# apple/ml-stable-diffusion

Hardware: AMD Instinct MI355X
Metric: diffusion iter/s (UNet steps/s), SD2.1-base 512x512 fp16 (higher is better)
Workload: dtype fp16; 1 GPU; BASELINE config 2: SD2.1-base (865.9 M-parameter UNet), random-init, denoising iteration at 512x512 (64x64 latents), CFG batch 2 per prompt, DDIM, device-resident loop; unet=sd21-base, latent=64, attention=ORIGINAL, prompts_per_gpu=1, global_batch=2, hip_graph=True, parallelism=dp1 (independent prompts per rank, no data-path collective)

## Files before the change

include/sd_mi355x.h:

```cpp
#ifndef SD_MI355X_H
#define SD_MI355X_H

#include <stddef.h>
#include <stdint.h>

#ifdef __cplusplus
extern "C" {
#endif

typedef enum sd_status {
  SD_OK = 0,
  SD_ERR_INVALID_ARGUMENT = -1,
  SD_ERR_NOT_FOUND = -2,
  SD_ERR_HIP = -3,
  SD_ERR_UNSUPPORTED = -4,
  SD_ERR_INTERNAL = -5
} sd_status;

typedef enum sd_dtype { SD_F16 = 0, SD_F32 = 1 } sd_dtype;

typedef enum sd_attention_impl {
  SD_ATTN_ORIGINAL = 0,
  SD_ATTN_SPLIT_EINSUM = 1,
  SD_ATTN_SPLIT_EINSUM_V2 = 2
// ... 140 lines not shown
                           const float* gn_bias, void* conv_out, void* out, int B, int Cin, int H, int W, int Cout, int ksize,
                           int groups, float eps, int silu, int tile, int producer_stats, int* entries, int iters, float* ms);
int sd_op_conv2d_groupnorm_proj(const void* x, const void* w, const float* bias, const void* res, const float* gn_weight,
                                const float* gn_bias, const void* proj_w, const float* proj_bias, void* conv_out, void* out, int B,
                                int Cin, int H, int W, int Cout, int ksize, int Nproj, int groups, float eps, int fold, int tile,
                                int* entries, int iters, float* ms);
int sd_op_conv2d_groupnorm_conv3x3(const void* x, const void* w, const float* bias, const void* res, const float* gn_weight,
                                   const float* gn_bias, const void* w2, const float* bias2, const void* res2, void* conv_out, void* out,
                                   int B, int Cin, int H, int W, int Cout, int ksize, int N2, int groups, float eps, int silu, int fold,
                                   int tile, int staging2, int* entries, int iters, float* ms);
int sd_op_ffn_out_proj(const void* g, const void* w1, const float* b1, const void* res1, const void* w2, const float* b2, const void* res2,
                       void* out, float* gn_sums, int B, int C, int S, int groups, int fused, int iters, float* ms);
int sd_op_fold_linear(const void* wp, const float* bp, const void* w2, const float* b2, void* wm_out, float* bm_out, int N, int J, int K);
int sd_op_cross_attention_fused(const void* x, const float* ln_weight, const float* ln_bias, const void* wq, const void* k,
                                const void* v, void* out, int B, int heads, int Sq, int Sk, float eps, int nst, int iters,
                                float* ms);
int sd_op_cross_attention_block(const void* x, const float* ln_weight, const float* ln_bias, const void* wq, const void* k, const void* v,
                                const void* wo, const float* bo, const void* a1, const void* wo1, const float* bo1, void* out, int B, int heads,
                                int Sq, int Sk, float eps, int fused, int iters, float* ms);
int sd_op_geglu(const void* x, const void* w, const float* bias, void* out, int M, int C, int N2, int iters, float* ms);
int sd_op_geglu_ln(const void* x, const float* ln_weight, const float* ln_bias, const void* w, const float* bias, void* out, int M, int C,
                   int N2, float eps, int kernel, int iters, float* ms);
int sd_op_qkv_ln(const void* x, const float* ln_weight, const float* ln_bias, const void* w, void* out_qk, void* out_vt, int B, int HW, int C,
                 float eps, float q_scale, int vt_perm, int kernel, int iters, float* ms);
int sd_op_gn_proj_qkv(const void* x_in, const void* conv_w, const float* gn_weight, const float* gn_bias, const void* proj_w,
                      const float* proj_bias, const float* ln_weight, const float* ln_bias, const void* wqkv, void* out_h, void* out_qk,
                      void* out_vt, int B, int H, int W, int C, int groups, float gn_eps, float ln_eps, float q_scale, int vt_perm, int fused,
                      int* entries, int iters, float* ms);
int sd_op_timestep_embedding(const float* t, float* out, int n, int dim, int flip_sin_to_cos, float freq_shift);
int sd_op_posterior_noise(const float* moments, const float* eps, const float* noise, float* out, int Cz, int h, int w, int n_images,
                          float scale_factor, float sa, float sb, int iters, float* ms);
int sd_op_conv_plan(int ksize, int stride, int up, int C0, int C1, int N, int B, int Ho, int Wo, int out_mode, int flags, int n_trans,
                    int n_twins, int gnf_groups, int tile, int staging, int splitk, int copies, int* plan, unsigned long long* workspace_bytes);
int sd_numpy_randn(uint32_t seed, double* out, size_t n);
int sd_torch_randn(uint32_t seed, double* out, size_t n);
int sd_philox_randn(uint64_t seed, uint32_t offset, double* out, size_t n);
int sd_calibrate(int device, float* out9);
int sd_selftest_mfma(void);

typedef struct sd_safety_checker_config {
  int32_t batch, image_size , patch_size , hidden_size, intermediate_size,
          num_hidden_layers, num_attention_heads, projection_dim, num_concepts ,
          num_special , hidden_act ;
  float layer_norm_eps;
  int32_t use_graph;
} sd_safety_checker_config;
typedef struct sd_safety_checker sd_safety_checker;
int sd_safety_checker_create(const sd_safety_checker_config* cfg, const sd_weights* w, int device, sd_safety_checker** out);
void sd_safety_checker_destroy(sd_safety_checker* c);
size_t sd_safety_checker_device_bytes(const sd_safety_checker* c);
int sd_safety_checker_run(sd_safety_checker* c, const void* clip_input, float adjustment, float* has_nsfw,
                          float* concept_scores, float* image_embeds, float* last_hidden_state, int flags);
float sd_safety_checker_last_ms(const sd_safety_checker* c);
int sd_op_vit_attention(const void* qkv, void* out, int B, int S, int heads, int d, int iters, float* ms);
int sd_op_safety_head(const float* image_embeds, const float* concept_embeds, const float* special_embeds,
                      const float* concept_w, const float* special_w, float adjustment, int B, int P,
                      int n_concepts, int n_special, float* has_nsfw, float* concept_scores);

#ifdef __cplusplus
}
#endif
#endif
```

ml-stable-diffusion_amd/csrc/capi_ops.cpp:

```cpp
#include <algorithm>
#include <climits>
#include <cmath>
#include <cstring>
#include <initializer_list>

#include "capi_util.h"
#include "conv_plan.h"
#include "weight_prep.h"

namespace sd {
namespace {

const half_t* f16(const void* p) { return reinterpret_cast<const half_t*>(p); }

half_t* upload_nhwc(Scratch& sc, const void* x, int B, int C, int H, int W) {
  const half_t* src = f16(x);
  std::vector<half_t> t((size_t)B * C * H * W);
  for (int b = 0; b < B; ++b)
    for (int c = 0; c < C; ++c)
      for (int p = 0; p < H * W; ++p) t[((size_t)b * H * W + p) * C + c] = src[((size_t)b * C + c) * H * W + p];
  return sc.dev<half_t>(t.size(), t.data());
}
half_t* upload_tokens(Scratch& sc, const void* x, int B, int C, int S) { return upload_nhwc(sc, x, B, C, 1, S); }

// ... 564 lines not shown
    cd.gnf_groups = groups;
    SD_REQUIRE(conv_fast_path_ok(cd), kInvalidArgument, "conv2d_groupnorm_conv3x3: the second conv must run on the MFMA path");
    const bool can_fold = fold && silu && conv_gn_loader_ok(cd);
    SD_REQUIRE(!fold || can_fold, kUnsupported, "conv2d_groupnorm_conv3x3: the halo loader cannot normalise C=%d groups=%d @%dx%d", Cout, groups, H, W);
    cd.gnf_groups = 0;
    ConvWorkspace ws = workspace_for(sc, {d, cd});
    int n_entries = 0;
    sc.timed(iters, ms, [&] {
      n_entries = launch_conv(d, ws, sc.stream);
      ConvDesc cc = cd;
      if (fold && n_entries >= 1 && n_entries <= 128) {
        fold_groupnorm(cc, dconv, partial, dgw, dgb, eps, groups, n_entries);
        cc.gnf_silu = silu ? 1 : 0;
      } else {
        launch_groupnorm(dconv, Cout, nullptr, 0, partial, dgw, dgb, dnorm, B, H * W, groups, eps, silu ? 1 : 0, sc.stream, n_entries);
        cc.x0 = dnorm;
      }
      launch_conv(cc, ws, sc.stream);
    });
    if (entries) *entries = (fold && n_entries >= 1 && n_entries <= 128) ? n_entries : 0;
    if (conv_out) download_nchw(dconv, conv_out, B, Cout, H, W);
    download_nchw(dy, out, B, N2, H, W);
  });
}

int sd_op_cross_attention_fused(const void* x, const float* ln_weight, const float* ln_bias, const void* wq, const void* k,
                                const void* v, void* out, int B, int heads, int Sq, int Sk, float eps, int nst, int iters,
                                float* ms) {
  return guarded([&] {
    SD_REQUIRE(x && ln_weight && ln_bias && wq && k && v && out, kInvalidArgument, "NULL argument");
    const int C = heads * 64;
    SD_REQUIRE(B > 0 && heads > 0 && xattn_fused_ok(C, heads, Sq, Sk), kUnsupported,
               "cross_attention_fused: heads %d x 64 channels, Sq %d, Sk %d (<= 96)", heads, Sq, Sk);
    Scratch sc;
    const int ldv = (Sk + 7) / 8 * 8;
    const FoldedProj fq = upload_ln_folded(sc, wq, nullptr, ln_weight, ln_bias, C, C, false);
    XAttnDesc d;
    d.x = upload_tokens(sc, x, B, C, Sq);
    d.wq = fq.w;
    d.bias = fq.bias;
    d.colsum = fq.colsum;
    d.k = upload_tokens(sc, k, B, C, Sk);
    d.vt = upload_vt(sc, v, B, C, Sk, ldv, false);
    half_t* o = sc.dev<half_t>((size_t)B * Sq * C);
    d.out = o;
    d.M = B * Sq; d.C = C; d.S = Sq; d.L = Sk; d.ldv = ldv; d.heads = heads;
    d.ln_eps = eps;
    d.nst = nst;
    sc.timed(iters, ms, [&] { launch_xattn_fused(d, sc.stream); });
    download_tokens(o, out, B, C, Sq);
  });
}

int sd_op_cross_attention_block(const void* x, const float* ln_weight, const float* ln_bias, const void* wq, const void* k, const void* v,
                                const void* wo, const float* bo, const void* a1, const void* wo1, const float* bo1, void* out, int B, int heads,
                                int Sq, int Sk, float eps, int fused, int iters, float* ms) {
  return guarded([&] {
    SD_REQUIRE(x && ln_weight && ln_bias && wq && k && v && wo && bo && out, kInvalidArgument, "NULL argument");
    const bool pre = a1 != nullptr;
    SD_REQUIRE(!pre || (wo1 && bo1), kInvalidArgument, "cross_attention_block: a1 needs wo1 and bo1");
    const int C = heads * 64;
    SD_REQUIRE(B > 0 && heads > 0 && xattn_fused_ok(C, heads, Sq, Sk), kUnsupported,
               "cross_attention_block: heads %d x 64 channels, Sq %d, Sk %d (<= 96)", heads, Sq, Sk);
    SD_REQUIRE(!fused || (xattn_out_ok(C, heads, Sq, Sk) && (!pre || heads == 5)), kUnsupported,
               "cross_attention_block: the one-launch form takes 5 or 10 heads (with a1: 5) and Sq %% 32 == 0 (heads %d, Sq %d)", heads, Sq);
    Scratch sc;
// ... 371 lines not shown
    ConvDesc d;
    d.x0 = d.w = ph;
    d.C0 = C0;
    if (C1 > 0) d.x1 = ph, d.C1 = C1;
    d.B = B; d.Ho = Ho; d.Wo = Wo; d.Hi = Ho * stride / up; d.Wi = Wo * stride / up;
    d.ksize = ksize; d.stride = stride; d.up = up; d.N = N; d.out_mode = out_mode;
    if (flags & 1) d.ln_colsum = present;
    if (flags & 2) d.temb = present;
    if (flags & 4) d.res = ph;
    if (flags & 8) d.gn_partial = const_cast<float*>(present), d.gn_groups = 32;
    if (flags & 16) d.bias = present;
    if (flags & 32) d.pad = 0;
    if (n_trans > 0) d.out_t = const_cast<half_t*>(ph), d.n_trans = n_trans, d.ldT = Ho * Wo;
    d.n_twins = n_twins;
    if (gnf_groups > 0) {
      d.gnf_partial = d.gnf_gamma = d.gnf_beta = present;
      d.gnf_groups = gnf_groups;
      d.gnf_entries = 1;
      d.gnf_silu = ksize == 3 ? 1 : 0;
    }
    d.tile = tile; d.staging = staging; d.splitk = splitk;
    const ConvWeightCopies c = conv_plan_copies(d);
    if (copies < 0) copies = (c.wstream ? 1 : 0) | (c.wsgemm ? 2 : 0) | (c.bvgemm ? 4 : 0);
    if (copies & 1) d.w_tiled = ph;
    if (copies & 2) d.w_ws = ph;
    if (copies & 4) d.w_bv = ph;
    const ConvPlan p = conv_plan(d);
    plan[0] = p.tile; plan[1] = p.staging; plan[2] = p.splitk; plan[3] = p.slab ? 1 : 0;
    plan[4] = c.wstream ? 1 : 0; plan[5] = c.wsgemm ? 1 : 0; plan[6] = c.bvgemm ? 1 : 0;
    *workspace_bytes = p.workspace_bytes;
  });
}

int sd_op_timestep_embedding(const float* t, float* out, int n, int dim, int flip_sin_to_cos, float freq_shift) {
  return guarded([&] {
    SD_REQUIRE(t && out && n > 0 && dim > 0 && dim % 2 == 0, kInvalidArgument, "bad arguments");
    SD_REQUIRE(flip_sin_to_cos == 1, kUnsupported, "flip_sin_to_cos=False is not on the path");
    Scratch sc;
    float* dt = sc.dev<float>(n, t);
    float* dout = sc.dev<float>((size_t)n * dim);
    std::vector<float> f = timestep_freq_table(dim, freq_shift);
    float* df = sc.dev<float>(f.size(), f.data());
    launch_timestep_embedding(dt, df, dout, n, dim, sc.stream);
    SD_HIP(hipStreamSynchronize(sc.stream));
    SD_HIP(hipMemcpy(out, dout, (size_t)n * dim * sizeof(float), hipMemcpyDeviceToHost));
  });
}

int sd_op_posterior_noise(const float* moments, const float* eps, const float* noise, float* out, int Cz, int h, int w, int n_images,
                          float scale_factor, float sa, float sb, int iters, float* ms) {
  return guarded([&] {
    SD_REQUIRE(moments && eps && noise && out, kInvalidArgument, "NULL argument");
    SD_REQUIRE(Cz > 0 && h > 0 && w > 0 && n_images > 0, kInvalidArgument, "posterior_noise: Cz=%d h=%d w=%d n_images=%d", Cz, h, w, n_images);
    Scratch sc;
    const size_t n = (size_t)Cz * h * w, total = (size_t)n_images * n, guard = 256;
    float* dm = sc.dev<float>(2 * n, moments);
    float* de = sc.dev<float>(n, eps);
    float* dn = sc.dev<float>(total, noise);
    float* dout = sc.dev<float>(total + guard);
    SD_HIP(hipMemset(dout, 0xff, (total + guard) * sizeof(float)));
    sc.timed(iters, ms, [&] { launch_posterior_noise(dm, de, dn, dout, n, n_images, scale_factor, sa, sb, sc.stream); });
    SD_HIP(hipStreamSynchronize(sc.stream));
    std::vector<uint32_t> g(guard);
    SD_HIP(hipMemcpy(g.data(), dout + total, guard * sizeof(float), hipMemcpyDeviceToHost));
    for (uint32_t v : g) SD_REQUIRE(v == 0xffffffffu, kInternal, "posterior_noise wrote behind its %zu outputs", total);
    SD_HIP(hipMemcpy(out, dout, total * sizeof(float), hipMemcpyDeviceToHost));
// ... 48 lines not shown
```

ml-stable-diffusion_amd/csrc/kernels.h:

```cpp
#pragma once
#include "sd_common.h"

namespace sd {

enum OutMode : int {
  kOutHalf = 0,
  kOutHalfT = 1,
  kOutGeglu = 2,
};

struct GnTwin {
  half_t* y = nullptr;
  int ld = 0, c_off = 0;
  int cpg = 0;
  const float* gamma = nullptr;
  const float* beta = nullptr;
  float eps = 1e-5f;
  int silu = 0;
};

struct ConvDesc {
  const half_t* x0 = nullptr;
  const half_t* x1 = nullptr;
  int C0 = 0, C1 = 0;
// ... 112 lines not shown
  int variant = 0;
  int vt_perm = 0;
  int q_prescaled = 0;
  float* sk_part = nullptr;
  size_t sk_part_bytes = 0;
  unsigned* sk_cnt = nullptr;
  int sk_cnt_n = 0;
  int sk_force = 0;
  int sk_upw = 0;
};
inline float attention_q_prescale(int d) { return 1.4426950408889634f / sqrtf((float)d); }
void launch_attention(const AttnDesc& d, hipStream_t s);
bool attention_supported(int d);
bool attention8_ok(const AttnDesc& d);
bool attention8_shape_ok(int d, int Sq, int Sk);
void launch_attention8(const AttnDesc& d, hipStream_t s);
bool attention8_sk_scratch(const AttnDesc& d, size_t* part_bytes, int* n_counters);

struct XAttnDesc {
  const half_t* x = nullptr;
  const half_t* wq = nullptr;
  const float* bias = nullptr;
  const float* colsum = nullptr;
  const half_t* k = nullptr;
  const half_t* vt = nullptr;
  half_t* out = nullptr;
  int M = 0, C = 0, S = 0, L = 0, ldv = 0, heads = 0;
  float ln_eps = 1e-5f;
  int impl = kAttnOriginal;
  int nst = 0;
};
bool xattn_fused_ok(int C, int heads, int S, int L);
void launch_xattn_fused(const XAttnDesc& d, hipStream_t s);

struct XAttnOutDesc {
  const half_t* x = nullptr;
  const half_t* wq_t = nullptr;
  const float* q_bias = nullptr;
  const float* q_colsum = nullptr;
  const half_t* k = nullptr;
  const half_t* vt = nullptr;
  const half_t* wo_t = nullptr;
  const float* o_bias = nullptr;
  half_t* out = nullptr;
  int M = 0, C = 0, S = 0, L = 0, ldv = 0, heads = 0;
  float ln_eps = 1e-5f;
  int impl = kAttnOriginal;
  const half_t* h0 = nullptr;
  const half_t* wo1_t = nullptr;
  const float* o1_bias = nullptr;
};
struct GnProjQkvDesc {
  const half_t* x = nullptr;
  const float* gn_partial = nullptr;
  const float* gn_gamma = nullptr;
  const float* gn_beta = nullptr;
  int gn_entries = 0, gn_groups = 32;
  float gn_eps = 1e-6f;
  const half_t* wp_t = nullptr;
  const float* p_bias = nullptr;
  half_t* h = nullptr;
  const half_t* wqkv_t = nullptr;
  const float* qkv_bias = nullptr;
  const float* qkv_colsum = nullptr;
  float ln_eps = 1e-5f;
  half_t* qk = nullptr;
// ... 112 lines not shown
```

ml-stable-diffusion_amd/csrc/xattn.hip:

```cpp
#include "kernels.h"

namespace sd {
namespace {

constexpr int BK = 64;
constexpr int XBM = 128;
constexpr int XD = 64;
constexpr int XKEYS = 96;
constexpr int KROW = XD + 4;
constexpr int VROW = XKEYS + 4;

struct XAttnArgs {
  const half_t* x;
  const half_t* wq;
  const float* bias;
  const float* colsum;
  const half_t* k;
  const half_t* vt;
  half_t* out;
  int M, C, S, L, ldv, heads;
  float ln_eps, scale_log2;
};

__device__ __forceinline__ float xor32_sumf(float v) {
  const unsigned u = __float_as_uint(v);
  const auto r = __builtin_amdgcn_permlane32_swap(u, u, false, false);
  const unsigned r0 = r[0], r1 = r[1];
  return __uint_as_float(r0) + __uint_as_float(r1);
}
__device__ __forceinline__ float xor32_maxf(float v) {
  const unsigned u = __float_as_uint(v);
  const auto r = __builtin_amdgcn_permlane32_swap(u, u, false, false);
  const unsigned r0 = r[0], r1 = r[1];
  return fmaxf(__uint_as_float(r0), __uint_as_float(r1));
}

constexpr size_t xattn_lds_bytes(int nst) {
  return (size_t)nst * (XBM + XD) * BK * 2 + (size_t)XKEYS * KROW * 2 + (size_t)XD * VROW * 2 + 2 * XD * sizeof(float);
}

template <int NST>
__global__ __launch_bounds__(256, xattn_lds_bytes(NST) <= 80 * 1024 ? 2 : 1) void xattn_fused_kernel(XAttnArgs a) {
  constexpr int XR = XBM / 32, WR = XD / 32;
  extern __shared__ __attribute__((aligned(16))) char smem[];
  half_t* Xs = reinterpret_cast<half_t*>(smem);
  half_t* Ws = Xs + NST * XBM * BK;
  half_t* Ks = Ws + NST * XD * BK;
  half_t* Vs = Ks + XKEYS * KROW;
  float* sconst = reinterpret_cast<float*>(Vs + XD * VROW);

  const int tid = threadIdx.x, lane = tid & 63;
  const int wave = __builtin_amdgcn_readfirstlane(tid >> 6);
  const int l31 = lane & 31, hi = lane >> 5;

  const int tps = (a.S + XBM - 1) / XBM;
  const int nwg = (a.M / a.S) * tps * a.heads;
  int bid = blockIdx.x;
  {
    const int q = nwg >> 3, r = nwg & 7, xcd = bid & 7, idx = bid >> 3;
    bid = ((xcd < r) ? xcd * (q + 1) : r * (q + 1) + (xcd - r) * q) + idx;
  }
  const int mt = bid / a.heads, h = bid - mt * a.heads;
  const int b = mt / tps;
  const int m_blk = b * a.S + (mt - b * tps) * XBM;
  const int rows_valid = min(XBM, a.S - (mt - b * tps) * XBM);
  const int nk = a.C / BK;

  const half8 zero8 = {0, 0, 0, 0, 0, 0, 0, 0};
  half8 kreg[3], vreg[3];
  {
    const half_t* kb = a.k + (size_t)b * a.L * a.C + (size_t)h * XD;
    const half_t* vb = a.vt + ((size_t)b * a.C + (size_t)h * XD) * a.ldv;
#pragma unroll
    for (int i = 0; i < 3; ++i) {
      const int idx = tid + i * 256;
      const int row = idx >> 3, ch = idx & 7;
      kreg[i] = (row < a.L) ? *reinterpret_cast<const half8*>(kb + (size_t)row * a.C + ch * 8) : zero8;
    }
#pragma unroll
    for (int i = 0; i < 3; ++i) {
      const int idx = tid + i * 256;
      const int row = idx / 12, ch = idx - row * 12;
      vreg[i] = (ch * 8 < a.ldv) ? *reinterpret_cast<const half8*>(vb + (size_t)row * a.ldv + ch * 8) : zero8;
    }
  }
  if (tid < XD) {
    sconst[tid] = a.bias[h * XD + tid];
    sconst[XD + tid] = a.colsum[h * XD + tid];
  }

  const int pchunk = tid & 7, lrow = tid >> 3;
  const int chunk = pchunk ^ ((lrow >> 1) & 7);
  const half_t* xp[XR];
  const half_t* wp[WR];
#pragma unroll
  for (int i = 0; i < XR; ++i) xp[i] = a.x + (size_t)min(m_blk + lrow + 32 * i, a.M - 1) * a.C + chunk * 8;
#pragma unroll
  for (int i = 0; i < WR; ++i) wp[i] = a.wq + (size_t)(h * XD + lrow + 32 * i) * a.C + chunk * 8;
  auto load_tile = [&](int stage) {
    char* xs = reinterpret_cast<char*>(Xs + stage * XBM * BK) + wave * 1024;
    char* ws = reinterpret_cast<char*>(Ws + stage * XD * BK) + wave * 1024;
#pragma unroll
    for (int i = 0; i < XR; ++i) {
      __builtin_amdgcn_global_load_lds((const __attribute__((address_space(1))) void*)xp[i],
                                       (__attribute__((address_space(3))) void*)(xs + i * 4096), 16, 0, 0);
      xp[i] += BK;
    }
#pragma unroll
    for (int i = 0; i < WR; ++i) {
      __builtin_amdgcn_global_load_lds((const __attribute__((address_space(1))) void*)wp[i],
                                       (__attribute__((address_space(3))) void*)(ws + i * 4096), 16, 0, 0);
      wp[i] += BK;
    }
  };

  floatx16 acc[2];
#pragma unroll
  for (int j = 0; j < 2; ++j)
#pragma unroll
    for (int r = 0; r < 16; ++r) acc[j][r] = 0.f;
  float ln_s1 = 0.f, ln_s2 = 0.f;
  const int fsw = (l31 >> 1) & 7;

  constexpr int PER_TILE = XR + WR;
  constexpr int DEPTH = NST - 2;
#pragma unroll
  for (int p = 0; p < NST - 1; ++p)
    if (p < nk) load_tile(p);
  for (int kt = 0; kt < nk; ++kt) {
    const int ahead = nk - 1 - kt;
    const int fly = ahead < DEPTH ? ahead : DEPTH;
    if (DEPTH >= 3 && fly == 3) asm volatile("s_waitcnt vmcnt(%0)\n\ts_barrier" ::"n"((DEPTH >= 3 ? 3 : 0) * PER_TILE) : "memory");
    else if (DEPTH >= 2 && fly == 2) asm volatile("s_waitcnt vmcnt(%0)\n\ts_barrier" ::"n"((DEPTH >= 2 ? 2 : 0) * PER_TILE) : "memory");
    else if (DEPTH >= 1 && fly == 1) asm volatile("s_waitcnt vmcnt(%0)\n\ts_barrier" ::"n"((DEPTH >= 1 ? 1 : 0) * PER_TILE) : "memory");
    else asm volatile("s_waitcnt vmcnt(0)\n\ts_barrier" ::: "memory");
    const int st = kt % NST;
    const half_t* xs = Xs + st * XBM * BK + (wave * 32 + l31) * BK;
    const half_t* ws = Ws + st * XD * BK + l31 * BK;
    half8 xf[4], wf[4][2];
#pragma unroll
    for (int kk = 0; kk < 4; ++kk) {
      const int koff = ((kk * 2 + hi) ^ fsw) * 8;
      xf[kk] = *reinterpret_cast<const half8*>(xs + koff);
#pragma unroll
      for (int j = 0; j < 2; ++j) wf[kk][j] = *reinterpret_cast<const half8*>(ws + j * 32 * BK + koff);
    }
    __builtin_amdgcn_sched_barrier(0);
    if (kt + NST - 1 < nk) load_tile((kt + NST - 1) % NST);
#pragma unroll
    for (int kk = 0; kk < 4; ++kk) {
#pragma unroll
      for (int j = 0; j < 2; ++j) acc[j] = __builtin_amdgcn_mfma_f32_32x32x16_f16(wf[kk][j], xf[kk], acc[j], 0, 0, 0);
      const half2v one2 = {(half_t)1.f, (half_t)1.f};
#pragma unroll
      for (int e = 0; e < 4; ++e) {
        const half2v p2 = {xf[kk][2 * e], xf[kk][2 * e + 1]};
        ln_s2 = __builtin_amdgcn_fdot2(p2, p2, ln_s2, false);
        ln_s1 = __builtin_amdgcn_fdot2(p2, one2, ln_s1, false);
      }
    }
  }

#pragma unroll
  for (int i = 0; i < 3; ++i) {
    const int idx = tid + i * 256;
    const int row = idx >> 3, ch = idx & 7;
    half_t* dst = Ks + row * KROW + ch * 8;
    *reinterpret_cast<half4*>(dst) = half4{kreg[i][0], kreg[i][1], kreg[i][2], kreg[i][3]};
    *reinterpret_cast<half4*>(dst + 4) = half4{kreg[i][4], kreg[i][5], kreg[i][6], kreg[i][7]};
  }
#pragma unroll
  for (int i = 0; i < 3; ++i) {
    const int idx = tid + i * 256;
    const int row = idx / 12, ch = idx - row * 12;
    half_t* dst = Vs + row * VROW + ch * 8;
    *reinterpret_cast<half4*>(dst) = half4{vreg[i][0], vreg[i][1], vreg[i][2], vreg[i][3]};
    *reinterpret_cast<half4*>(dst + 4) = half4{vreg[i][4], vreg[i][5], vreg[i][6], vreg[i][7]};
  }
  __syncthreads();

  half8 qf[2][2];
  {
    const float inv_k = 1.0f / (float)a.C;
    const float s1 = xor32_sumf(ln_s1), s2 = xor32_sumf(ln_s2);
    const float mean = s1 * inv_k;
    const float var = fmaxf(s2 * inv_k - mean * mean, 0.f);
    const float ln_a = rsqrtf(var + a.ln_eps);
    const float ln_b = -ln_a * mean;
#pragma unroll
    for (int j = 0; j < 2; ++j)
#pragma unroll
      for (int q4 = 0; q4 < 4; ++q4) {
        const int nl = j * 32 + 8 * q4 + 4 * hi;
        const floatx4 bb = *reinterpret_cast<const floatx4*>(sconst + nl);
        const floatx4 cs = *reinterpret_cast<const floatx4*>(sconst + XD + nl);
#pragma unroll
        for (int e = 0; e < 4; ++e) {
          const int r = 4 * q4 + e;
          qf[j][r >> 3][r & 7] = (half_t)fmaf(acc[j][r], ln_a, fmaf(ln_b, cs[e], bb[e]));
        }
      }
  }

  floatx16 sacc[3];
#pragma unroll
  for (int kt = 0; kt < 3; ++kt) {
#pragma unroll
    for (int r = 0; r < 16; ++r) sacc[kt][r] = 0.f;
    const half_t* kr = Ks + (kt * 32 + l31) * KROW + 4 * hi;
#pragma unroll
    for (int j = 0; j < 2; ++j)
#pragma unroll
// ... 18 lines not shown
  float ps4[4] = {0.f, 0.f, 0.f, 0.f};
#pragma unroll
  for (int kt = 0; kt < 3; ++kt)
#pragma unroll
    for (int r = 0; r < 16; ++r) {
      const float p = __builtin_amdgcn_exp2f(fmaf(sacc[kt][r], a.scale_log2, -mnew));
      sacc[kt][r] = p;
      ps4[r & 3] += p;
    }
  const float inv = 1.0f / xor32_sumf((ps4[0] + ps4[1]) + (ps4[2] + ps4[3]));

  floatx16 oacc[2];
#pragma unroll
  for (int ct = 0; ct < 2; ++ct)
#pragma unroll
    for (int r = 0; r < 16; ++r) oacc[ct][r] = 0.f;
#pragma unroll
  for (int kt = 0; kt < 3; ++kt)
#pragma unroll
    for (int s2 = 0; s2 < 2; ++s2) {
      half8 pf;
#pragma unroll
      for (int e = 0; e < 8; ++e) pf[e] = (half_t)sacc[kt][s2 * 8 + e];
#pragma unroll
      for (int ct = 0; ct < 2; ++ct) {
        const half_t* vp = Vs + (ct * 32 + l31) * VROW + kt * 32 + s2 * 16 + 4 * hi;
        const half4 v0 = *reinterpret_cast<const half4*>(vp);
        const half4 v1 = *reinterpret_cast<const half4*>(vp + 8);
        const half8 vf = {v0[0], v0[1], v0[2], v0[3], v1[0], v1[1], v1[2], v1[3]};
        oacc[ct] = __builtin_amdgcn_mfma_f32_32x32x16_f16(vf, pf, oacc[ct], 0, 0, 0);
      }
    }

  if (wave * 32 + l31 >= rows_valid) return;
  half_t* orow = a.out + (size_t)(m_blk + wave * 32 + l31) * a.C + (size_t)h * XD;
#pragma unroll
  for (int ct = 0; ct < 2; ++ct)
#pragma unroll
    for (int g = 0; g < 4; ++g) {
      const half4 o = {(half_t)(oacc[ct][4 * g] * inv), (half_t)(oacc[ct][4 * g + 1] * inv),
                       (half_t)(oacc[ct][4 * g + 2] * inv), (half_t)(oacc[ct][4 * g + 3] * inv)};
      *reinterpret_cast<half4*>(orow + ct * 32 + 8 * g + 4 * hi) = o;
    }
}

template <int NST>
void launch_nst(const XAttnArgs& a, hipStream_t s) {
  constexpr size_t lds = xattn_lds_bytes(NST);
  static_assert(lds <= 160 * 1024, "LDS");
  auto k = xattn_fused_kernel<NST>;
  static DynLdsOnce once;
  once.set(k, lds);
  hipLaunchKernelGGL(k, dim3((a.M / a.S) * ((a.S + XBM - 1) / XBM) * a.heads), dim3(256), lds, s, a);
}

}

bool xattn_fused_ok(int C, int heads, int S, int L) {
  static const bool off = tune_env_set("SD_NO_XATTN_FUSED");
  return !off && heads >= 1 && C == heads * XD && C % BK == 0 && S >= 1 && L >= 1 && L <= XKEYS;
}

void launch_xattn_fused(const XAttnDesc& d, hipStream_t s) {
  SD_REQUIRE(xattn_fused_ok(d.C, d.heads, d.S, d.L), kInvalidArgument, "xattn_fused: C=%d heads=%d S=%d L=%d", d.C, d.heads, d.S,
             d.L);
  SD_REQUIRE(d.M % d.S == 0 && d.ldv % 8 == 0 && d.ldv >= d.L && d.ldv <= XKEYS, kInvalidArgument, "xattn_fused: M=%d ldv=%d", d.M,
             d.ldv);
  if (d.impl == kAttnSplitEinsumV2 && d.S >= 512)
    SD_REQUIRE(d.S % 512 == 0, kInvalidArgument, "SPLIT_EINSUM_V2 needs S_q %% 512 == 0 (got %d)", d.S);
  XAttnArgs a{d.x, d.wq, d.bias, d.colsum, d.k, d.vt, d.out, d.M, d.C, d.S, d.L, d.ldv, d.heads, d.ln_eps,
              1.4426950408889634f / sqrtf((float)XD)};
  static const int forced = tune_env_int("SD_XATTN_NST", 0);
  const int nst = forced ? forced : (d.nst ? d.nst : (d.C <= 640 ? 2 : 3));
  if (nst >= 5) launch_nst<5>(a, s);
  else if (nst == 4) launch_nst<4>(a, s);
  else if (nst == 3) launch_nst<3>(a, s);
  else launch_nst<2>(a, s);
  SD_HIP(hipGetLastError());
}

}
```

ml-stable-diffusion_amd/python_hip_stable_diffusion/_lib.py:

```python
import ctypes as C
import os

import numpy as np

_HERE = os.path.dirname(os.path.abspath(__file__))
LIB_PATH = os.environ.get("SD_MI355X_LIB", os.path.join(os.path.dirname(_HERE), "lib", "libsdmi355.so"))

SD_MAX_LEVELS = 6
SD_FLAG_DEVICE_PTRS = 1
ATTENTION_IMPLEMENTATIONS = {"ORIGINAL": 0, "SPLIT_EINSUM": 1, "SPLIT_EINSUM_V2": 2}


class LibraryNotBuilt(ImportError):
    pass


class UNetConfig(C.Structure):
    _fields_ = [
        ("batch", C.c_int32), ("in_channels", C.c_int32), ("out_channels", C.c_int32),
        ("height", C.c_int32), ("width", C.c_int32), ("n_levels", C.c_int32),
        ("block_out_channels", C.c_int32 * SD_MAX_LEVELS),
        ("down_cross_attn", C.c_int32 * SD_MAX_LEVELS),
        ("up_cross_attn", C.c_int32 * SD_MAX_LEVELS),
        ("layers_per_block", C.c_int32),
# ... 74 lines not shown
    ("sd_vae_encode", _I, [_P, _P, _I, _FP, _I]),
    ("sd_vae_encode_latents", _I, [_P, _P, _I, _FP, _FP, _I, _F, _F, _F, _FP, _I]),
    ("sd_text_encoder_create", _I, [_P, _P, _I, C.POINTER(_P)]),
    ("sd_text_encoder_destroy", None, [_P]),
    ("sd_text_encoder_device_bytes", C.c_size_t, [_P]),
    ("sd_text_encoder_encode", _I, [_P, C.POINTER(C.c_int32), _I, _FP, _FP, _FP]),
    ("sd_op_attention", _I, [_I, _P, _P, _P, _P, _I, _I, _I, _I, _I, _I, _I, _FP]),
    ("sd_op_layernorm", _I, [_P, _FP, _FP, _P, _I, _I, _I, _F, _I, _FP]),
    ("sd_op_groupnorm", _I, [_P, _FP, _FP, _P, _I, _I, _I, _I, _I, _F, _I, _I, _FP]),
    ("sd_op_groupnorm_shortcut", _I, [_P, _P, _FP, _FP, _P, _FP, _P, _P, _I, _I, _I, _I, _I, _I, _I, _F, _I, _I, _I, _FP]),
    ("sd_op_conv2d", _I, [_P, _P, _FP, _P, _P, _I, _I, _I, _I, _I, _I, _I, _I, _I, _I, _I, _I, _FP]),
    ("sd_op_conv2d_ex", _I, [_P, _P, _P, _FP, _FP, _P, _P, _I, _I, _I, _I, _I, _I, _I, _I, _I, _I, _I, _FP, _FP, _F, _I, _P, _I, _I, _I,
                             C.POINTER(_I), _I, _FP]),
    ("sd_op_conv2d_palettized", _I, [_P, _P, _P, _I, _P, _FP, _P, _P, _I, _I, _I, _I, _I, _I, _I, _I, _I, C.POINTER(_I), _I, _FP]),
    ("sd_op_palette_pack", _I, [_P, _I, _I, _I, _I, _P, C.POINTER(C.c_size_t)]),
    ("sd_op_gemm_palettized", _I, [_P, _P, _I, _P, _FP, _P, _P, _I, _I, _I, _I, _I, _I, C.POINTER(_I), _I, _FP]),
    ("sd_op_palette_pack_gemm", _I, [_P, _I, _I, _I, _P, C.POINTER(C.c_size_t)]),
    ("sd_op_conv2d_groupnorm", _I, [_P, _P, _FP, _P, _FP, _FP, _P, _P, _I, _I, _I, _I, _I, _I, _I, _F, _I, _I, _I, C.POINTER(_I), _I, _FP]),
    ("sd_op_conv2d_groupnorm_proj", _I, [_P, _P, _FP, _P, _FP, _FP, _P, _FP, _P, _P, _I, _I, _I, _I, _I, _I, _I, _I, _F, _I, _I, C.POINTER(_I), _I, _FP]),
    ("sd_op_conv2d_groupnorm_conv3x3", _I, [_P, _P, _FP, _P, _FP, _FP, _P, _FP, _P, _P, _P, _I, _I, _I, _I, _I, _I, _I, _I, _F, _I, _I, _I, _I,
                                            C.POINTER(_I), _I, _FP]),
    ("sd_op_cross_attention_fused", _I, [_P, _FP, _FP, _P, _P, _P, _P, _I, _I, _I, _I, _F, _I, _I, _FP]),
    ("sd_op_ffn_out_proj", _I, [_P, _P, _FP, _P, _P, _FP, _P, _P, _FP, _I, _I, _I, _I, _I, _I, _FP]),
    ("sd_op_fold_linear", _I, [_P, _FP, _P, _FP, _P, _FP, _I, _I, _I]),
    ("sd_op_cross_attention_block", _I, [_P, _FP, _FP, _P, _P, _P, _P, _FP, _P, _P, _FP, _P, _I, _I, _I, _I, _F, _I, _I, _FP]),
    ("sd_op_geglu", _I, [_P, _P, _FP, _P, _I, _I, _I, _I, _FP]),
    ("sd_op_geglu_ln", _I, [_P, _FP, _FP, _P, _FP, _P, _I, _I, _I, C.c_float, _I, _I, _FP]),
    ("sd_op_qkv_ln", _I, [_P, _FP, _FP, _P, _P, _P, _I, _I, _I, C.c_float, C.c_float, _I, _I, _I, _FP]),
    ("sd_op_gn_proj_qkv", _I, [_P, _P, _FP, _FP, _P, _FP, _FP, _FP, _P, _P, _P, _P, _I, _I, _I, _I, _I, C.c_float, C.c_float, C.c_float, _I, _I,
                               C.POINTER(C.c_int), _I, _FP]),
    ("sd_op_timestep_embedding", _I, [_FP, _FP, _I, _I, _I, _F]),
    ("sd_op_posterior_noise", _I, [_FP, _FP, _FP, _FP, _I, _I, _I, _I, _F, _F, _F, _I, _FP]),
    ("sd_op_conv_plan", _I, [_I] * 18 + [C.POINTER(C.c_int), C.POINTER(C.c_ulonglong)]),
    ("sd_numpy_randn", _I, [C.c_uint32, C.POINTER(C.c_double), C.c_size_t]),
    ("sd_torch_randn", _I, [C.c_uint32, C.POINTER(C.c_double), C.c_size_t]),
    ("sd_philox_randn", _I, [C.c_uint64, C.c_uint32, C.POINTER(C.c_double), C.c_size_t]),
    ("sd_calibrate", _I, [_I, _FP]),
    ("sd_selftest_mfma", _I, []),
    ("sd_safety_checker_create", _I, [C.POINTER(SafetyCheckerConfig), _P, _I, C.POINTER(_P)]),
    ("sd_safety_checker_destroy", None, [_P]),
    ("sd_safety_checker_device_bytes", C.c_size_t, [_P]),
    ("sd_safety_checker_last_ms", C.c_float, [_P]),
    ("sd_safety_checker_run", _I, [_P, _P, _F, _FP, _FP, _FP, _FP, _I]),
    ("sd_op_vit_attention", _I, [_P, _P, _I, _I, _I, _I, _I, _FP]),
    ("sd_op_safety_head", _I, [_FP, _FP, _FP, _FP, _FP, _F, _I, _I, _I, _I, _FP, _FP]),
]


def lib():
    global _lib
    if _lib is not None:
        return _lib
    if not os.path.exists(LIB_PATH):
        raise LibraryNotBuilt(
            f"{LIB_PATH} is missing - build it with `python -c 'import __graft_entry__ as g; g.build()'` "
            f"or `make -C ml-stable-diffusion_amd/csrc`. There is no CPU fallback.")
    if not os.environ.get("SD_MI355X_NO_TORCH"):
        try:
            import torch
        except Exception:
            pass
    handle = C.CDLL(LIB_PATH, mode=C.RTLD_GLOBAL)
    for name, restype, argtypes in SYMBOLS:
        fn = getattr(handle, name)
        fn.restype = restype
        fn.argtypes = argtypes
# ... 436 lines not shown
    out_qk = np.empty((M, 2 * Cn), np.float16)
    out_vt = np.empty((batch, Cn, HW), np.float16)
    ms = C.c_float(0)
    check(lib().sd_op_qkv_ln(ptr(x), fptr(f32(ln_weight)), fptr(f32(ln_bias)), ptr(w), ptr(out_qk), ptr(out_vt), batch, HW, Cn, eps, q_scale,
                             int(vt_perm), kernel, iters, C.byref(ms)))
    return out_qk, out_vt, ms.value


def gn_proj_qkv(x_in, conv_w, gn_weight, gn_bias, proj_w, proj_bias, ln_weight, ln_bias, wqkv, groups=32, gn_eps=1e-6, ln_eps=1e-5,
                q_scale=1.0, vt_perm=True, fused=True, iters=1):
    x_in, conv_w, proj_w, wqkv = f16(x_in), f16(conv_w), f16(proj_w), f16(wqkv)
    B, Cn, H, W = x_in.shape
    M = B * H * W
    h = np.empty((M, Cn), np.float16)
    qk = np.empty((M, 2 * Cn), np.float16)
    vt = np.empty((B, Cn, H * W), np.float16)
    ms, entries = C.c_float(0), C.c_int(0)
    check(lib().sd_op_gn_proj_qkv(ptr(x_in), ptr(conv_w), fptr(f32(gn_weight)), fptr(f32(gn_bias)), ptr(proj_w), fptr(f32(proj_bias)),
                                  fptr(f32(ln_weight)), fptr(f32(ln_bias)), ptr(wqkv), ptr(h), ptr(qk), ptr(vt), B, H, W, Cn, groups, gn_eps,
                                  ln_eps, q_scale, int(vt_perm), int(fused), C.byref(entries), iters, C.byref(ms)))
    return h, qk, vt, entries.value, ms.value


def conv_plan(ksize, stride, up, C0, C1, N, B, Ho, Wo, out_mode=0, flags=0, n_trans=0, n_twins=0, gnf_groups=0, tile=0, staging=0, splitk=0,
              copies=-1):
    plan = (C.c_int * 7)()
    ws = C.c_ulonglong(0)
    check(lib().sd_op_conv_plan(ksize, stride, up, C0, C1, N, B, Ho, Wo, out_mode, flags, n_trans, n_twins, gnf_groups, tile, staging, splitk,
                                copies, plan, C.byref(ws)))
    return {"tile": plan[0], "staging": plan[1], "splitk": plan[2], "slab": bool(plan[3]), "workspace_bytes": int(ws.value),
            "copies": (bool(plan[4]), bool(plan[5]), bool(plan[6]))}


def timestep_embedding(t, dim, flip_sin_to_cos=True, freq_shift=0.0):
    t = f32(t)
    out = np.empty((t.shape[0], dim), np.float32)
    check(lib().sd_op_timestep_embedding(fptr(t), fptr(out), t.shape[0], dim, int(flip_sin_to_cos), freq_shift))
    return out


def posterior_noise(moments, eps, noise, scale_factor, sa, sb, iters=1):
    moments, eps, noise = f32(moments), f32(eps), f32(noise)
    if noise.ndim != 4:
        raise ValueError("posterior_noise: noise must be (n_images, Cz, h, w)")
    n_images, Cz, h, w = noise.shape
    if moments.size != 2 * Cz * h * w or moments.shape[-3:] != (2 * Cz, h, w) or eps.shape[-3:] != (Cz, h, w) or eps.size != Cz * h * w:
        raise ValueError("posterior_noise: moments must be (2*Cz, h, w) and eps (Cz, h, w) for noise (n_images, Cz, h, w)")
    out = np.empty_like(noise)
    ms = C.c_float(0)
    check(lib().sd_op_posterior_noise(fptr(moments), fptr(eps), fptr(noise), fptr(out), Cz, h, w, n_images, float(scale_factor), float(sa),
                                      float(sb), iters, C.byref(ms)))
    return out, ms.value


def numpy_randn(seed, n):
    out = np.empty(n, np.float64)
    check(lib().sd_numpy_randn(seed, out.ctypes.data_as(C.POINTER(C.c_double)), n))
    return out


def torch_randn(seed, n):
    out = np.empty(n, np.float64)
    check(lib().sd_torch_randn(seed, out.ctypes.data_as(C.POINTER(C.c_double)), n))
    return out


# ... 13 lines not shown
```

Baseline: 244.4 it/s.

## Plan cross-attention fused kernel tiles: 64-token tile with K-split waves for small grids

Adds a planner for the fused cross-attention kernel. When the work-group count fits the CU count, it picks a 64-token tile with deeper staging and splits the K reduction across wave pairs, exchanging partial sums through LDS. It also adds tile-order selection (heads-fastest versus token-fastest) with magic-number division in place of the fixed XCD remap, and clamps K/V loads so they no longer branch. The aim is to fill more CUs on the low-resolution UNet levels, where 128-token tiles launch too few work-groups. The cost is extra LDS exchange and synchronisation, plus more template variants to compile.

Result: no change. 246.4 it/s, median of 6 (+0.8%).

```diff
diff --git a/include/sd_mi355x.h b/include/sd_mi355x.h
--- a/include/sd_mi355x.h
+++ b/include/sd_mi355x.h
@@ -196,6 +196,7 @@
                           float scale_factor, float sa, float sb, int iters, float* ms);
 int sd_op_conv_plan(int ksize, int stride, int up, int C0, int C1, int N, int B, int Ho, int Wo, int out_mode, int flags, int n_trans,
                     int n_twins, int gnf_groups, int tile, int staging, int splitk, int copies, int* plan, unsigned long long* workspace_bytes);
+int sd_op_xattn_plan(int C, int heads, int S, int B, int code, int* plan, unsigned long long* lds_bytes);
 int sd_numpy_randn(uint32_t seed, double* out, size_t n);
 int sd_torch_randn(uint32_t seed, double* out, size_t n);
 int sd_philox_randn(uint64_t seed, uint32_t offset, double* out, size_t n);
diff --git a/ml-stable-diffusion_amd/csrc/capi_ops.cpp b/ml-stable-diffusion_amd/csrc/capi_ops.cpp
--- a/ml-stable-diffusion_amd/csrc/capi_ops.cpp
+++ b/ml-stable-diffusion_amd/csrc/capi_ops.cpp
@@ -620,6 +620,7 @@
     const int C = heads * 64;
     SD_REQUIRE(B > 0 && heads > 0 && xattn_fused_ok(C, heads, Sq, Sk), kUnsupported,
                "cross_attention_fused: heads %d x 64 channels, Sq %d, Sk %d (<= 96)", heads, Sq, Sk);
+    xattn_plan(C, heads, Sq, B, nst);
     Scratch sc;
     const int ldv = (Sk + 7) / 8 * 8;
     const FoldedProj fq = upload_ln_folded(sc, wq, nullptr, ln_weight, ln_bias, C, C, false);
@@ -1057,6 +1058,15 @@
   });
 }
 
+int sd_op_xattn_plan(int C, int heads, int S, int B, int code, int* plan, unsigned long long* lds_bytes) {
+  return guarded([&] {
+    SD_REQUIRE(plan && lds_bytes, kInvalidArgument, "NULL argument");
+    const XAttnPlan p = xattn_plan(C, heads, S, B, code);
+    plan[0] = p.token_tile; plan[1] = p.stages; plan[2] = p.grid;
+    *lds_bytes = p.lds_bytes;
+  });
+}
+
 int sd_op_timestep_embedding(const float* t, float* out, int n, int dim, int flip_sin_to_cos, float freq_shift) {
   return guarded([&] {
     SD_REQUIRE(t && out && n > 0 && dim > 0 && dim % 2 == 0, kInvalidArgument, "bad arguments");
diff --git a/ml-stable-diffusion_amd/csrc/kernels.h b/ml-stable-diffusion_amd/csrc/kernels.h
--- a/ml-stable-diffusion_amd/csrc/kernels.h
+++ b/ml-stable-diffusion_amd/csrc/kernels.h
@@ -168,6 +168,13 @@
 };
 bool xattn_fused_ok(int C, int heads, int S, int L);
 void launch_xattn_fused(const XAttnDesc& d, hipStream_t s);
+constexpr int kXAttnPlanCus = 256;
+struct XAttnPlan {
+  int token_tile = 0, stages = 0, grid = 0;
+  size_t lds_bytes = 0;
+  bool legacy = false;
+};
+XAttnPlan xattn_plan(int C, int heads, int S, int B, int code, int cus = kXAttnPlanCus);
 
 struct XAttnOutDesc {
   const half_t* x = nullptr;
diff --git a/ml-stable-diffusion_amd/csrc/xattn.hip b/ml-stable-diffusion_amd/csrc/xattn.hip
--- a/ml-stable-diffusion_amd/csrc/xattn.hip
+++ b/ml-stable-diffusion_amd/csrc/xattn.hip
@@ -1,10 +1,15 @@
+#include <algorithm>
+#include <atomic>
+
+#include "conv_plan.h"
 #include "kernels.h"
+#include "sm_ring.h"
+#include "sm_tile.h"
 
 namespace sd {
 namespace {
 
 constexpr int BK = 64;
-constexpr int XBM = 128;
 constexpr int XD = 64;
 constexpr int XKEYS = 96;
 constexpr int KROW = XD + 4;
@@ -20,6 +25,9 @@
   half_t* out;
   int M, C, S, L, ldv, heads;
   float ln_eps, scale_log2;
+  SmTileOrder order;
+  unsigned grid_q, grid_r;
+  unsigned tps, tps_magic;
 };
 
 __device__ __forceinline__ float xor32_sumf(float v) {
@@ -35,13 +43,18 @@
   return fmaxf(__uint_as_float(r0), __uint_as_float(r1));
 }
 
-constexpr size_t xattn_lds_bytes(int nst) {
-  return (size_t)nst * (XBM + XD) * BK * 2 + (size_t)XKEYS * KROW * 2 + (size_t)XD * VROW * 2 + 2 * XD * sizeof(float);
-}
-
-template <int NST>
-__global__ __launch_bounds__(256, xattn_lds_bytes(NST) <= 80 * 1024 ? 2 : 1) void xattn_fused_kernel(XAttnArgs a) {
+constexpr size_t xattn_lds_bytes(int xbm, int nst) {
+  return (size_t)nst * (xbm + XD) * BK * 2 + (size_t)XKEYS * KROW * 2 + (size_t)XD * VROW * 2 + 2 * XD * sizeof(float);
+}
+
+template <int XBM, int NST>
+__global__ __launch_bounds__(256, xattn_lds_bytes(XBM, NST) <= 80 * 1024 ? 2 : 1) void xattn_fused_kernel(XAttnArgs a) {
+  static_assert(XBM == 128 || XBM == 64, "token tile");
   constexpr int XR = XBM / 32, WR = XD / 32;
+  constexpr int TW = XBM / 32;
+  constexpr int KH = 4 / TW;
+  constexpr int KSTEPS = 4 / KH;
+  static_assert((size_t)NST * (XBM + XD) * BK * 2 >= (KH - 1) * TW * 34 * 64 * sizeof(float), "the K-half exchange fits the ring");
   extern __shared__ __attribute__((aligned(16))) char smem[];
   half_t* Xs = reinterpret_cast<half_t*>(smem);
   half_t* Ws = Xs + NST * XBM * BK;
@@ -52,18 +65,22 @@
   const int tid = threadIdx.x, lane = tid & 63;
   const int wave = __builtin_amdgcn_readfirstlane(tid >> 6);
   const int l31 = lane & 31, hi = lane >> 5;
-
-  const int tps = (a.S + XBM - 1) / XBM;
-  const int nwg = (a.M / a.S) * tps * a.heads;
-  int bid = blockIdx.x;
-  {
-    const int q = nwg >> 3, r = nwg & 7, xcd = bid & 7, idx = bid >> 3;
-    bid = ((xcd < r) ? xcd * (q + 1) : r * (q + 1) + (xcd - r) * q) + idx;
-  }
-  const int mt = bid / a.heads, h = bid - mt * a.heads;
-  const int b = mt / tps;
-  const int m_blk = b * a.S + (mt - b * tps) * XBM;
-  const int rows_valid = min(XBM, a.S - (mt - b * tps) * XBM);
+  const int tw = wave % TW, kh = wave / TW;
+
+  int mt, h;
+  if (a.grid_r == 0) {
+    sm_tile_coords(a.order, mt, h);
+  } else {
+    const unsigned xcd = blockIdx.x & 7u, idx = blockIdx.x >> 3;
+    const unsigned t = ((xcd < a.grid_r) ? xcd * (a.grid_q + 1) : a.grid_r * (a.grid_q + 1) + (xcd - a.grid_r) * a.grid_q) + idx;
+    const unsigned slow = __umulhi(t, a.order.fast_magic), fast = t - slow * a.order.fast_div;
+    mt = (int)(a.order.n_fast ? slow : fast);
+    h = (int)(a.order.n_fast ? fast : slow);
+  }
+  const int b = a.tps == 1 ? mt : (int)__umulhi((unsigned)mt, a.tps_magic);
+  const int tile_in_sample = mt - b * (int)a.tps;
+  const int m_blk = b * a.S + tile_in_sample * XBM;
+  const int rows_valid = min(XBM, a.S - tile_in_sample * XBM);
   const int nk = a.C / BK;
 
   const half8 zero8 = {0, 0, 0, 0, 0, 0, 0, 0};
@@ -75,19 +92,16 @@
     for (int i = 0; i < 3; ++i) {
       const int idx = tid + i * 256;
       const int row = idx >> 3, ch = idx & 7;
-      kreg[i] = (row < a.L) ? *reinterpret_cast<const half8*>(kb + (size_t)row * a.C + ch * 8) : zero8;
+      kreg[i] = *reinterpret_cast<const half8*>(kb + (size_t)min(row, a.L - 1) * a.C + ch * 8);
     }
 #pragma unroll
     for (int i = 0; i < 3; ++i) {
       const int idx = tid + i * 256;
       const int row = idx / 12, ch = idx - row * 12;
-      vreg[i] = (ch * 8 < a.ldv) ? *reinterpret_cast<const half8*>(vb + (size_t)row * a.ldv + ch * 8) : zero8;
-    }
-  }
-  if (tid < XD) {
-    sconst[tid] = a.bias[h * XD + tid];
-    sconst[XD + tid] = a.colsum[h * XD + tid];
-  }
+      vreg[i] = *reinterpret_cast<const half8*>(vb + (size_t)row * a.ldv + min(ch * 8, a.ldv - 8));
+    }
+  }
+  const float sconst_v = ((tid & XD) ? a.colsum : a.bias)[h * XD + (tid & (XD - 1))];
 
   const int pchunk = tid & 7, lrow = tid >> 3;
   const int chunk = pchunk ^ ((lrow >> 1) & 7);
@@ -122,25 +136,21 @@
   float ln_s1 = 0.f, ln_s2 = 0.f;
   const int fsw = (l31 >> 1) & 7;
 
-  constexpr int PER_TILE = XR + WR;
+  constexpr int PPW = XR + WR;
   constexpr int DEPTH = NST - 2;
+  static_assert(PPW * DEPTH <= 63, "vmcnt range");
 #pragma unroll
   for (int p = 0; p < NST - 1; ++p)
     if (p < nk) load_tile(p);
   for (int kt = 0; kt < nk; ++kt) {
-    const int ahead = nk - 1 - kt;
-    const int fly = ahead < DEPTH ? ahead : DEPTH;
-    if (DEPTH >= 3 && fly == 3) asm volatile("s_waitcnt vmcnt(%0)\n\ts_barrier" ::"n"((DEPTH >= 3 ? 3 : 0) * PER_TILE) : "memory");
-    else if (DEPTH >= 2 && fly == 2) asm volatile("s_waitcnt vmcnt(%0)\n\ts_barrier" ::"n"((DEPTH >= 2 ? 2 : 0) * PER_TILE) : "memory");
-    else if (DEPTH >= 1 && fly == 1) asm volatile("s_waitcnt vmcnt(%0)\n\ts_barrier" ::"n"((DEPTH >= 1 ? 1 : 0) * PER_TILE) : "memory");
-    else asm volatile("s_waitcnt vmcnt(0)\n\ts_barrier" ::: "memory");
+    sm_wait<PPW, 0, DEPTH>(min(DEPTH, nk - 1 - kt));
     const int st = kt % NST;
-    const half_t* xs = Xs + st * XBM * BK + (wave * 32 + l31) * BK;
+    const half_t* xs = Xs + st * XBM * BK + (tw * 32 + l31) * BK;
     const half_t* ws = Ws + st * XD * BK + l31 * BK;
-    half8 xf[4], wf[4][2];
-#pragma unroll
-    for (int kk = 0; kk < 4; ++kk) {
-      const int koff = ((kk * 2 + hi) ^ fsw) * 8;
+    half8 xf[KSTEPS], wf[KSTEPS][2];
+#pragma unroll
+    for (int kk = 0; kk < KSTEPS; ++kk) {
+      const int koff = (((kh * KSTEPS + kk) * 2 + hi) ^ fsw) * 8;
       xf[kk] = *reinterpret_cast<const half8*>(xs + koff);
 #pragma unroll
       for (int j = 0; j < 2; ++j) wf[kk][j] = *reinterpret_cast<const half8*>(ws + j * 32 * BK + koff);
@@ -148,7 +158,7 @@
     __builtin_amdgcn_sched_barrier(0);
     if (kt + NST - 1 < nk) load_tile((kt + NST - 1) % NST);
 #pragma unroll
-    for (int kk = 0; kk < 4; ++kk) {
+    for (int kk = 0; kk < KSTEPS; ++kk) {
 #pragma unroll
       for (int j = 0; j < 2; ++j) acc[j] = __builtin_amdgcn_mfma_f32_32x32x16_f16(wf[kk][j], xf[kk], acc[j], 0, 0, 0);
       const half2v one2 = {(half_t)1.f, (half_t)1.f};
@@ -166,18 +176,42 @@
     const int idx = tid + i * 256;
     const int row = idx >> 3, ch = idx & 7;
     half_t* dst = Ks + row * KROW + ch * 8;
-    *reinterpret_cast<half4*>(dst) = half4{kreg[i][0], kreg[i][1], kreg[i][2], kreg[i][3]};
-    *reinterpret_cast<half4*>(dst + 4) = half4{kreg[i][4], kreg[i][5], kreg[i][6], kreg[i][7]};
+    const half8 kv = row < a.L ? kreg[i] : zero8;
+    *reinterpret_cast<half4*>(dst) = half4{kv[0], kv[1], kv[2], kv[3]};
+    *reinterpret_cast<half4*>(dst + 4) = half4{kv[4], kv[5], kv[6], kv[7]};
   }
 #pragma unroll
   for (int i = 0; i < 3; ++i) {
     const int idx = tid + i * 256;
     const int row = idx / 12, ch = idx - row * 12;
     half_t* dst = Vs + row * VROW + ch * 8;
-    *reinterpret_cast<half4*>(dst) = half4{vreg[i][0], vreg[i][1], vreg[i][2], vreg[i][3]};
-    *reinterpret_cast<half4*>(dst + 4) = half4{vreg[i][4], vreg[i][5], vreg[i][6], vreg[i][7]};
-  }
-  __syncthreads();
+    const half8 vv = ch * 8 < a.ldv ? vreg[i] : zero8;
+    *reinterpret_cast<half4*>(dst) = half4{vv[0], vv[1], vv[2], vv[3]};
+    *reinterpret_cast<half4*>(dst + 4) = half4{vv[4], vv[5], vv[6], vv[7]};
+  }
+  if (tid < 2 * XD) sconst[tid] = sconst_v;
+  if constexpr (KH == 2) {
+    float* xch = reinterpret_cast<float*>(smem) + tw * 64 + lane;
+    __syncthreads();
+    if (kh == 1) {
+#pragma unroll
+      for (int j = 0; j < 2; ++j)
+#pragma unroll
+        for (int r = 0; r < 16; ++r) xch[(j * 16 + r) * TW * 64] = acc[j][r];
+      xch[32 * TW * 64] = ln_s1;
+      xch[33 * TW * 64] = ln_s2;
+    }
+    __syncthreads();
+    if (kh == 1) return;
+#pragma unroll
+    for (int j = 0; j < 2; ++j)
+#pragma unroll
+      for (int r = 0; r < 16; ++r) acc[j][r] += xch[(j * 16 + r) * TW * 64];
+    ln_s1 += xch[32 * TW * 64];
+    ln_s2 += xch[33 * TW * 64];
+  } else {
+    __syncthreads();
+  }
 
   half8 qf[2][2];
   {
@@ -262,8 +296,8 @@
       }
     }
 
-  if (wave * 32 + l31 >= rows_valid) return;
-  half_t* orow = a.out + (size_t)(m_blk + wave * 32 + l31) * a.C + (size_t)h * XD;
+  if (tw * 32 + l31 >= rows_valid) return;
+  half_t* orow = a.out + (size_t)(m_blk + tw * 32 + l31) * a.C + (size_t)h * XD;
 #pragma unroll
   for (int ct = 0; ct < 2; ++ct)
 #pragma unroll
@@ -274,14 +308,51 @@
     }
 }
 
-template <int NST>
-void launch_nst(const XAttnArgs& a, hipStream_t s) {
-  constexpr size_t lds = xattn_lds_bytes(NST);
+template <int XBM, int NST>
+void launch_form(const XAttnArgs& a, int grid, hipStream_t s) {
+  constexpr size_t lds = xattn_lds_bytes(XBM, NST);
   static_assert(lds <= 160 * 1024, "LDS");
-  auto k = xattn_fused_kernel<NST>;
+  auto k = xattn_fused_kernel<XBM, NST>;
   static DynLdsOnce once;
   once.set(k, lds);
-  hipLaunchKernelGGL(k, dim3((a.M / a.S) * ((a.S + XBM - 1) / XBM) * a.heads), dim3(256), lds, s, a);
+  hipLaunchKernelGGL(k, dim3(grid), dim3(256), lds, s, a);
+}
+
+template <int XBM, int NST = (XBM == 64 ? 8 : 5)>
+void launch_depth(const XAttnArgs& a, int stages, int grid, hipStream_t s) {
+  if constexpr (NST > 2) {
+    if (stages < NST) return launch_depth<XBM, NST - 1>(a, stages, grid, s);
+  }
+  launch_form<XBM, NST>(a, grid, s);
+}
+
+void xattn_order(XAttnArgs& a, int B, int tps, int grid, bool heads_fastest) {
+  const unsigned mt = (unsigned)(B * tps), nt = (unsigned)a.heads;
+  SmTileOrder o;
+  o.per_xcd = (unsigned)grid / 8;
+  o.n_fast = heads_fastest ||
+             choose_tile_order(2.0 * a.M * a.C, 2.0 * a.C * a.C + 2.0 * B * a.C * (a.L + a.ldv), (double)mt, (double)nt, false);
+  if ((o.n_fast ? nt : mt) == 1) o.n_fast = !o.n_fast;
+  o.fast_div = o.n_fast ? nt : mt;
+  o.fast_magic = (unsigned)((1ull << 32) / o.fast_div + 1);
+  a.order = o;
+  a.grid_q = (unsigned)grid >> 3;
+  a.grid_r = (unsigned)grid & 7;
+  a.tps = (unsigned)tps;
+  a.tps_magic = (unsigned)((1ull << 32) / a.tps + 1);
+}
+
+int current_device_cus() {
+  static std::atomic<int> cus[64];
+  int dev = 0;
+  SD_HIP(hipGetDevice(&dev));
+  if (dev < 0 || dev >= 64) return kXAttnPlanCus;
+  int v = cus[dev].load(std::memory_order_relaxed);
+  if (v == 0) {
+    if (hipDeviceGetAttribute(&v, hipDeviceAttributeMultiprocessorCount, dev) != hipSuccess || v <= 0) v = kXAttnPlanCus;
+    cus[dev].store(v, std::memory_order_relaxed);
+  }
+  return v;
 }
 
 }
@@ -291,7 +362,36 @@
   return !off && heads >= 1 && C == heads * XD && C % BK == 0 && S >= 1 && L >= 1 && L <= XKEYS;
 }
 
+bool xattn_code_ok(int code) { return code == 0 || (code >= 2 && code <= 5) || (code >= 62 && code <= 68); }
+
+XAttnPlan xattn_plan(int C, int heads, int S, int B, int code, int cus) {
+  SD_REQUIRE(xattn_code_ok(code), kInvalidArgument, "xattn_fused: code %d (0, 2-5: 128-token tile, 62-68: 64-token tile)", code);
+  SD_REQUIRE(heads >= 1 && C == heads * XD && S >= 1 && B >= 1 && cus >= 1, kInvalidArgument, "xattn_plan: C=%d heads=%d S=%d B=%d", C,
+             heads, S, B);
+  static const bool small_off = tune_env_int("SD_XATTN_SMALL", 1) == 0;
+  const int nk = C / BK;
+  auto grid_of = [&](int tile) { return (long long)B * cdiv(S, tile) * heads; };
+  XAttnPlan p;
+  if (code >= 62) {
+    p.token_tile = 64, p.stages = code - 60;
+  } else if (code >= 2) {
+    p.token_tile = 128, p.stages = code;
+  } else if (!small_off && grid_of(64) <= cus) {
+    p.token_tile = 64, p.stages = std::max(2, std::min(8, nk));
+  } else if (!small_off && grid_of(128) <= cus) {
+    p.token_tile = 128, p.stages = std::max(2, std::min(5, nk));
+  } else {
+    p.token_tile = 128, p.stages = C <= 640 ? 2 : 3;
+  }
+  SD_REQUIRE(grid_of(p.token_tile) <= 0x7fffffff, kInvalidArgument, "xattn_plan: grid");
+  p.grid = (int)grid_of(p.token_tile);
+  p.lds_bytes = xattn_lds_bytes(p.token_tile, p.stages);
+  p.legacy = code == 0 && small_off;
+  return p;
+}
+
 void launch_xattn_fused(const XAttnDesc& d, hipStream_t s) {
+  SD_REQUIRE(xattn_code_ok(d.nst), kInvalidArgument, "xattn_fused: code %d", d.nst);
   SD_REQUIRE(xattn_fused_ok(d.C, d.heads, d.S, d.L), kInvalidArgument, "xattn_fused: C=%d heads=%d S=%d L=%d", d.C, d.heads, d.S,
              d.L);
   SD_REQUIRE(d.M % d.S == 0 && d.ldv % 8 == 0 && d.ldv >= d.L && d.ldv <= XKEYS, kInvalidArgument, "xattn_fused: M=%d ldv=%d", d.M,
@@ -301,11 +401,11 @@
   XAttnArgs a{d.x, d.wq, d.bias, d.colsum, d.k, d.vt, d.out, d.M, d.C, d.S, d.L, d.ldv, d.heads, d.ln_eps,
               1.4426950408889634f / sqrtf((float)XD)};
   static const int forced = tune_env_int("SD_XATTN_NST", 0);
-  const int nst = forced ? forced : (d.nst ? d.nst : (d.C <= 640 ? 2 : 3));
-  if (nst >= 5) launch_nst<5>(a, s);
-  else if (nst == 4) launch_nst<4>(a, s);
-  else if (nst == 3) launch_nst<3>(a, s);
-  else launch_nst<2>(a, s);
+  const int B = d.M / d.S;
+  const XAttnPlan p = xattn_plan(d.C, d.heads, d.S, B, forced ? std::max(2, std::min(5, forced)) : d.nst, current_device_cus());
+  xattn_order(a, B, cdiv(d.S, p.token_tile), p.grid, p.legacy);
+  if (p.token_tile == 64) launch_depth<64>(a, p.stages, p.grid, s);
+  else launch_depth<128>(a, p.stages, p.grid, s);
   SD_HIP(hipGetLastError());
 }
 
diff --git a/ml-stable-diffusion_amd/python_hip_stable_diffusion/_lib.py b/ml-stable-diffusion_amd/python_hip_stable_diffusion/_lib.py
--- a/ml-stable-diffusion_amd/python_hip_stable_diffusion/_lib.py
+++ b/ml-stable-diffusion_amd/python_hip_stable_diffusion/_lib.py
@@ -130,6 +130,7 @@
     ("sd_op_timestep_embedding", _I, [_FP, _FP, _I, _I, _I, _F]),
     ("sd_op_posterior_noise", _I, [_FP, _FP, _FP, _FP, _I, _I, _I, _I, _F, _F, _F, _I, _FP]),
     ("sd_op_conv_plan", _I, [_I] * 18 + [C.POINTER(C.c_int), C.POINTER(C.c_ulonglong)]),
+    ("sd_op_xattn_plan", _I, [_I] * 5 + [C.POINTER(C.c_int), C.POINTER(C.c_ulonglong)]),
     ("sd_numpy_randn", _I, [C.c_uint32, C.POINTER(C.c_double), C.c_size_t]),
     ("sd_torch_randn", _I, [C.c_uint32, C.POINTER(C.c_double), C.c_size_t]),
     ("sd_philox_randn", _I, [C.c_uint64, C.c_uint32, C.POINTER(C.c_double), C.c_size_t]),
@@ -632,6 +633,13 @@
             "copies": (bool(plan[4]), bool(plan[5]), bool(plan[6]))}
 
 
+def xattn_plan(C_, heads, S, B, code=0):
+    plan = (C.c_int * 3)()
+    lds = C.c_ulonglong(0)
+    check(lib().sd_op_xattn_plan(C_, heads, S, B, code, plan, C.byref(lds)))
+    return {"token_tile": plan[0], "stages": plan[1], "grid": plan[2], "lds_bytes": int(lds.value)}
+
+
 def timestep_embedding(t, dim, flip_sin_to_cos=True, freq_shift=0.0):
     t = f32(t)
     out = np.empty((t.shape[0], dim), np.float32)
```
